# tikroeger/OF_DIS

Measured on AMD Instinct MI355X. Metric: frames/sec at 1024×436 op-point-2 (INT), higher is better.
Workload: dtype f32

## Files before the change

### of_dis_amd/csrc/ofdis_fused.hip

```cpp
#include <stdlib.h>

#include "ofdis_fused.h"

namespace ofdis {
namespace OFDIS_KNS {

constexpr int MW_LAG = 8;
constexpr int MW_MAX_ITERS = 8;
constexpr int MW_RING = 8;
constexpr int SP_LAG = 9;
constexpr int SP_MAX_ITERS = 6;


template <int NS, bool BRIGHT, int MODE, int NOC = 1>
__global__ __launch_bounds__(MODE == 2 ? 128 * SP_MAX_ITERS : (MODE == 1 ? 64 * MW_MAX_ITERS : 256))
__attribute__((amdgpu_waves_per_eu(NOC == 3 ? 2 : (MODE == 1 ? 3 : 1)))) void tv_fused_kernel(const FusedArgs a, const int R) {
  constexpr int U = 6;
  constexpr bool MW = MODE != 0;
  constexpr int MAXIT = MODE == 2 ? SP_MAX_ITERS : MW_MAX_ITERS;
  __shared__ float2 xring[MW ? (MAXIT - 1) * MW_RING * 64 : 1];
  __shared__ float sring[MODE == 2 ? SP_MAX_ITERS * 2 * SLOT_FLOATS * 64 : 1];
  __shared__ float2 wdring[MODE == 1 ? 6 * 64 : 1];
  __shared__ float2 obring[MODE == 1 ? 6 * 64 : 1];
  constexpr int PDW = 5, PDD = NOC == 3 ? 2 : 3;
  constexpr int PDU = MODE == 2 ? 4 : (MODE == 1 ? 3 : PDW);
  constexpr int LAG = MODE == 2 ? SP_LAG : MW_LAG;
  static_assert(2 * (NS - 1) + 1 < U, "slot ring too small for this many pipelined sweeps");
  static_assert(!MW || LAG >= PDU + 2 * (NS - 1) + 1, "a row must be published before the next iteration reads it");
  const int w = a.t.w, h = a.t.h;
  const int rw = a.S * w;
  const int lane = threadIdx.x & 63;
  const int wv = MW ? __builtin_amdgcn_readfirstlane(threadIdx.x >> 6) : 0;
  const int n_iters = MODE == 2 ? (int)(blockDim.x >> 7) : (MW ? (int)(blockDim.x >> 6) : 1);
  const bool is_solver = MODE == 2 && wv >= n_iters;
  const int it = MODE == 2 ? (is_solver ? wv - n_iters : wv) : wv;
  const bool do_p = MODE != 2 || !is_solver;
  const bool do_s = MODE != 2 || is_solver;
  const int wid = MW ? (int)blockIdx.x : __builtin_amdgcn_readfirstlane(blockIdx.x * 4 + (threadIdx.x >> 6));
  const int G = 64 / R;
  const int nstrips = a.t.nframes / a.S;
  const int s0 = wid * G;
  if (s0 >= nstrips) return;
  int fl = lane / R;
  const int jr = lane % R;
  const bool row_ok = (s0 + fl < nstrips) && (jr < h);
  if (s0 + fl >= nstrips) fl = nstrips - 1 - s0;
  const int j = jr < h ? jr : h - 1;
  const bool has_top = j > 0, has_bot = j < h - 1;
  const float omega = a.omega, qa = a.quarter_alpha, hd3 = a.half_delta_over3, hg3 = a.half_gamma_over3;
  auto from_prev = [&](float x) { return wave_from_prev(x); };
  auto from_next = [&](float x) { return wave_from_next(x); };

  const int nst = min(G, nstrips - s0);
  const size_t strip_recs = (size_t)rw * h;
  auto rsrc = [&](const float* base, int rec_floats) {
    return __builtin_amdgcn_make_buffer_rsrc((void*)(base + (size_t)s0 * strip_recs * rec_floats), 0,
                                             (int)(nst * strip_recs * rec_floats * 4), 0x00020000);
  };
  const __amdgpu_buffer_rsrc_t rsW = rsrc(a.wrec, 2), rsU = rsrc(a.uv, 2);
  const __amdgpu_buffer_rsrc_t rsD = rsrc(a.d8, 8);
  const __amdgpu_buffer_rsrc_t rsD1 = rsrc(a.d8 + (NOC == 3 ? (size_t)a.t.nframes * w * h * 8 : 0), 8);
  const __amdgpu_buffer_rsrc_t rsD2 = rsrc(a.d8 + (NOC == 3 ? (size_t)a.t.nframes * w * h * 16 : 0), 8);
  const int vrec = fl * (int)strip_recs + j;
  const int vo8 = vrec * 32, vo2 = vrec * 8;
  auto asf = [](unsigned u) { return __builtin_bit_cast(float, u); };

  const int npx = w * h;
  float2* const flow_row = a.flow_out
                               ? reinterpret_cast<float2*>(a.flow_out) + ((size_t)(s0 + fl) * a.S * npx + (size_t)j * w)
                               : nullptr;
  const bool aos_out = MODE != 2 && a.flow_out != nullptr;

  FRow W[6];
  FDer D[PDD][NOC];
  float uu[3], vv[3], sm[3];
  FSlot slot[6];
#pragma unroll
  for (int r = 0; r < 6; ++r) { W[r] = FRow{0, 0, 0, 0}; slot[r] = FSlot{1, 0, 1, 0, 0, 1, 1, 0, 0, 0, 0}; }
#pragma unroll
  for (int r = 0; r < 3; ++r) {
    uu[r] = vv[r] = 0.0f;
    sm[r] = 1.0f;
  }
#pragma unroll
  for (int r = 0; r < PDD; ++r)
#pragma unroll
    for (int c = 0; c < NOC; ++c) D[r][c] = FDer{0, 0, 0, 0, 0, 0, 0, 0};
  float ru[NS], rv[NS], ru2[NS], rv2[NS];
#pragma unroll
  for (int s = 0; s < NS; ++s) { ru[s] = rv[s] = ru2[s] = rv2[s] = 0.0f; }
  float ldx = 0.0f, ldy = 0.0f;
  float2 Wd[6], ob[U];
#pragma unroll
  for (int r = 0; r < 6; ++r) Wd[r] = make_float2(0.0f, 0.0f);
#pragma unroll
  for (int r = 0; r < U; ++r) ob[r] = make_float2(0.0f, 0.0f);
  int ox = 0, ooff = 0;

  auto ob_put = [&](int e, const float2& v) {
    if constexpr (MODE == 1) obring[lane * U + e] = v;
    else ob[e] = v;
  };
  auto ob_get = [&](int e) -> float2 {
    if constexpr (MODE == 1) return obring[lane * U + e];
    else return ob[e];
  };
  auto aos_emit = [&](int slot, bool flush, const float2& wq, float du, float dv, int c) {
    ob_put(slot, make_float2(wq.x + du, wq.y + dv));
    if (flush) {
      const int c0 = c - (U - 1);
      if (row_ok & (c0 >= 0) & (c < rw) & (ox >= U - 1)) {
        typedef float f4a8 __attribute__((ext_vector_type(4), aligned(8)));
        f4a8* d = reinterpret_cast<f4a8*>(flow_row + ooff + ox - (U - 1));
#pragma unroll
        for (int e = 0; e < U / 2; ++e) {
          const float2 p0 = ob_get(2 * e), p1 = ob_get(2 * e + 1);
          d[e] = f4a8{p0.x, p0.y, p1.x, p1.y};
        }
      } else if (row_ok & (c >= 0) & (c0 < rw)) {
#pragma unroll
        for (int e = 0; e < U; ++e) {
          const int ce = c0 + e;
          int xe = ox - (U - 1) + e, oe = ooff;
          if (xe < 0) { xe += w; oe -= npx; }
          if ((ce >= 0) & (ce < rw)) flow_row[oe + xe] = ob_get(e);
        }
      }
    }
    if (c >= 0) {
      ++ox;
      if (ox == w) { ox = 0; ooff += npx; }
    }
  };
  auto wrap_row = [&](int r) { r %= rw; return r < 0 ? r + rw : r; };
  auto wrap_col = [&](int c) { c %= w; return c < 0 ? c + w : c; };
  auto next_row = [&](int r) { return (r + 1 == rw) ? 0 : r + 1; };
  auto ring_uv = [&](FRow& r, int tau) {
    if (it == 0) {
      r.du = 0.0f; r.dv = 0.0f;
    } else {
      const float2 v = xring[((it - 1) * MW_RING + (tau & (MW_RING - 1))) * 64 + lane];
      r.du = v.x; r.dv = v.y;
    }
  };
  auto load_w = [&](FRow& r, int drow, int tau, bool zero_uv) {
    const int o = drow * h * 8;
    const auto t = __builtin_amdgcn_raw_buffer_load_b64(rsW, vo2, o, 0);
    const unsigned t0 = t[0], t1 = t[1];
    r.wx = asf(t0); r.wy = asf(t1);
    if constexpr (MODE == 0) {
      const auto q = __builtin_amdgcn_raw_buffer_load_b64(rsU, zero_uv ? 0x7ffffff0 : vo2, o, 0);
      const unsigned q0 = q[0], q1 = q[1];
      r.du = asf(q0); r.dv = asf(q1);
    }
  };
  auto load_d1 = [&](FDer& r, const __amdgpu_buffer_rsrc_t& rs, int o) {
    const auto lo = __builtin_amdgcn_raw_buffer_load_b128(rs, vo8, o, 0);
    const auto hi = __builtin_amdgcn_raw_buffer_load_b128(rs, vo8 + 16, o, 0);
    const unsigned l0 = lo[0], l1 = lo[1], l2 = lo[2], l3 = lo[3], h0 = hi[0], h1 = hi[1], h2 = hi[2], h3 = hi[3];
    r.ix = asf(l0); r.iz = asf(l1); r.ixx = asf(l2); r.ixz = asf(l3);
    r.iy = asf(h0); r.ixy = asf(h1); r.iyz = asf(h2); r.iyy = asf(h3);
  };
  auto load_d = [&](FDer (&r)[NOC], int drow) {
    const int o = drow * h * 32;
    load_d1(r[0], rsD, o);
    if constexpr (NOC == 3) {
      load_d1(r[1], rsD1, o);
      load_d1(r[2], rsD2, o);
    }
  };

  if constexpr (MW) {
    if (do_s && it < MAXIT - 1) {
#pragma unroll
      for (int q = 0; q < MW_RING; ++q) xring[(it * MW_RING + q) * 64 + lane] = make_float2(0.0f, 0.0f);
    }
    __syncthreads();
    for (int n = 0; n < it * LAG; ++n) __syncthreads();
  }
  if (do_p) {
    load_w(W[2], wrap_row(-1), -1, true);
    load_w(W[3], wrap_row(0), 0, true);
    if (PDW == 5) load_w(W[4], wrap_row(1), 1, true);
    if constexpr (MW) {
      ring_uv(W[2], -1);
      if (PDU == 4) ring_uv(W[3], 0);
    }
  }
  int rowW = wrap_row(PDW - 3);
  int tauW = PDW - 3;
  int rowD = wrap_row(PDD - 3);
  int srow = wrap_row(-3 - 2 * (NS - 1));
  int x2 = wrap_col(-1 - j);
  bool x1_last = (wrap_col(-2 - j) == w - 1);

  const int wtot = (MW ? 1 : a.n_inner) * rw;
  const int tend = (wtot - 1) + (h - 1) + 2 * (NS - 1);
  int ig = -3 - j - 2 * (NS - 1);
  bool first_w = !MW;
  int taus = -3 - 2 * (NS - 1);
  int taut = -3;
  for (int k0 = 0; k0 <= tend + 3; k0 += U) {
#pragma unroll
    for (int u = 0; u < U; ++u) {
      if (do_p) {
        load_w(W[(u + PDW) % 6], rowW, tauW, first_w);
        if constexpr (MW) ring_uv(W[(u + PDU) % 6], tauW - (PDW - PDU));
        rowW = next_row(rowW);
        ++tauW;
        load_d(D[(u + PDD) % PDD], rowD);
        rowD = next_row(rowD);
        {
          const FRow& r = W[(u + 3) % 6];
          uu[u % 3] = r.wx + r.du;
          vv[u % 3] = r.wy + r.dv;
        }
        const bool x2_last = (x2 == w - 1);
        {
          const float uc = uu[(u + 2) % 3], vc = vv[(u + 2) % 3];
          float ul = uu[(u + 1) % 3], vl = vv[(u + 1) % 3];
          float ur = uu[u % 3], vr = vv[u % 3];
          float ut = from_prev(uu[(u + 1) % 3]), vt = from_prev(vv[(u + 1) % 3]);
          float ub = from_next(uu[u % 3]), vb = from_next(vv[u % 3]);
          if (x2 == 0) { ul = uc; vl = vc; }
          if (x2_last) { ur = uc; vr = vc; }
          if (!has_top) { ut = uc; vt = vc; }
          if (!has_bot) { ub = uc; vb = vc; }
          const float ex = ur - ul, fx = vr - vl, ey = ub - ut, fy = vb - vt;
          sm[(u + 2) % 3] = fdiv_by_sqrt(qa, 0.25f * (ex * ex + ey * ey + fx * fx + fy * fy) + EPS_SMOOTH);
        }
        {
          const float sc = sm[(u + 1) % 3];
          const float s_r = sm[(u + 2) % 3];
          const float sh_c = x1_last ? 0.0f : sc + s_r;
          const FRow& rc = W[(u + 1) % 6];
          const FRow& rm = W[u % 6];
          const FRow& rp = W[(u + 2) % 6];
          float a11, a12, a22, b1, b2;
          if constexpr (NOC == 1) data_term_gray<BRIGHT>(D[(u + 1) % PDD][0], rc.du, rc.dv, hd3, hg3, a11, a12, a22, b1, b2);
          else data_term_rgb<BRIGHT>(D[(u + 1) % PDD], rc.du, rc.dv, hd3, hg3, a11, a12, a22, b1, b2);
          float udx, udy, ddx, ddy, sv_s;
          vertical_terms(udx, udy, ddx, ddy, sv_s, rc.wx, rc.wy, rm.wx, rm.wy, rp.wx, rp.wy, sc, sm[(u + 2) % 3]);
          const float sv_c = has_bot ? sv_s : 0.0f;
          const float sh_l = slot[u % 6].sh;
          const float sv_t = from_prev(slot[u % 6].sv);
          const float rdx = rp.wx - rc.wx, rdy = rp.wy - rc.wy;
          b1 -= sh_l * ldx;
          b2 -= sh_l * ldy;
          b1 += sh_c * rdx;
          b2 += sh_c * rdy;
          ldx = rdx; ldy = rdy;
          if constexpr (MODE == 0) Wd[(u + 1) % 6] = make_float2(rc.wx, rc.wy);
          if constexpr (MODE == 1) {
            if (it == n_iters - 1) wdring[((u + 1) % 6) * 64 + lane] = make_float2(rc.wx, rc.wy);
          }
          b1 -= sv_t * udx;
          b2 -= sv_t * udy;
          b1 += sv_c * ddx;
          b2 += sv_c * ddy;
          FSlot& o = slot[(u + 1) % 6];
          o.a11 = a11; o.a12 = a12; o.a22 = a22; o.b1 = b1; o.b2 = b2; o.sh = sh_c; o.sv = sv_c;
          o.dur = rp.du; o.dvr = rp.dv;
          o.hl = sh_l; o.vt = sv_t;
          if constexpr (MODE == 2) {
            float* sr = sring + ((it * 2 + ((taut + 1) & 1)) * SLOT_FLOATS) * 64 + lane;
            sr[0 * 64] = a11; sr[1 * 64] = a12; sr[2 * 64] = a22; sr[3 * 64] = b1; sr[4 * 64] = b2; sr[5 * 64] = sh_c;
            sr[6 * 64] = sv_c; sr[7 * 64] = rp.du; sr[8 * 64] = rp.dv; sr[9 * 64] = sh_l; sr[10 * 64] = sv_t;
          }
        }
        x1_last = x2_last;
        x2 = x2_last ? 0 : x2 + 1;
      }
      if (do_s) {
        if (MODE == 2 && taut > -3) {
          const float* sr = sring + ((it * 2 + (taut & 1)) * SLOT_FLOATS) * 64 + lane;
          FSlot& c = slot[u % 6];
          c.a11 = sr[0 * 64]; c.a12 = sr[1 * 64]; c.a22 = sr[2 * 64]; c.b1 = sr[3 * 64]; c.b2 = sr[4 * 64]; c.sh = sr[5 * 64];
          c.sv = sr[6 * 64]; c.dur = sr[7 * 64]; c.dvr = sr[8 * 64]; c.hl = sr[9 * 64]; c.vt = sr[10 * 64];
        }
        {
          FSlot& c = slot[u % 6];
          const float d = c.hl + c.sh + c.vt + c.sv;
          const float A11 = c.a22 + d, A22 = c.a11 + d;
          const float det = A11 * A22 - c.a12 * c.a12;
          const FDen dd = fden(det);
          c.a11 = fdiv_by(A11, dd);
          c.a22 = fdiv_by(A22, dd);
          c.a12 = -fdiv_by(c.a12, dd);
        }
        float nu[NS], nv[NS], ou[NS], ov[NS], rgu[NS], rgv[NS], wvt[NS], wsv[NS], s1[NS], s2[NS];
#pragma unroll
        for (int s = 0; s < NS; ++s) {
          const FSlot& c = slot[(u - 2 * s + 12) % 6];
          if (s == 0) {
            const FSlot& p = slot[(u + 5) % 6];
            ou[s] = p.dur; ov[s] = p.dvr;
            rgu[s] = c.dur; rgv[s] = c.dvr;
          } else {
            ou[s] = ru2[s - 1]; ov[s] = rv2[s - 1];
            rgu[s] = ru[s - 1]; rgv[s] = rv[s - 1];
          }
          wvt[s] = c.vt; wsv[s] = c.sv;
        }
        mul_pairs_from_prev(s1, s2, ru, rv, wvt);
#pragma unroll
        for (int s = 0; s < NS; ++s) {
          const FSlot& c = slot[(u - 2 * s + 12) % 6];
          s1[s] = c.sh * rgu[s] + s1[s];
          s2[s] = c.sh * rgv[s] + s2[s];
        }
        fmac_pairs_from_next(s1, s2, rgu, rgv, wsv);
#pragma unroll
        for (int s = 0; s < NS; ++s) {
          const FSlot& c = slot[(u - 2 * s + 12) % 6];
          const float lu = ru[s], lv = rv[s];
          const float t1 = s1[s] + c.b1, t2 = s2[s] + c.b2;
          const float B1 = c.hl * lu + t1, B2 = c.hl * lv + t2;
          nu[s] = ou[s] + omega * (c.a11 * B1 + c.a12 * B2 - ou[s]);
          nv[s] = ov[s] + omega * (c.a12 * B1 + c.a22 * B2 - ov[s]);
        }
        {
          if (!MW) {
            const int cw = ig + (PDW + 1 + 2 * (NS - 1));
            first_w = (cw < rw) | (cw >= wtot);
          }
          if (MW && it < n_iters - 1) {
            xring[(it * MW_RING + (taus & (MW_RING - 1))) * 64 + lane] = make_float2(nu[NS - 1], nv[NS - 1]);
          } else if (MODE == 2 && a.flow_out) {
            const auto q = __builtin_amdgcn_raw_buffer_load_b64(rsW, vo2, srow * h * 8, 0);
            const unsigned q0 = q[0], q1 = q[1];
            if (row_ok && ig >= 0 && ig < wtot)
              flow_row[ig] = make_float2(asf(q0) + nu[NS - 1], asf(q1) + nv[NS - 1]);
          } else if (MODE == 1 && a.flow_out) {
            aos_emit(u, u == U - 1, wdring[((u - 2 * (NS - 1) + 12) % 6) * 64 + lane], nu[NS - 1], nv[NS - 1], ig);
          } else if (!MW) {
            const u32x2 v = {__builtin_bit_cast(unsigned, nu[NS - 1]), __builtin_bit_cast(unsigned, nv[NS - 1])};
            const int lastc = ig - (wtot - rw);
            const bool on = row_ok & (ig >= 0) & (aos_out ? lastc < 0 : ig < wtot);
            __builtin_amdgcn_raw_buffer_store_b64(v, rsU, on ? vo2 : 0x7ffffff0, srow * h * 8, 0);
            if (aos_out) aos_emit(u, u == U - 1, Wd[(u - 2 * (NS - 1) + 12) % 6], nu[NS - 1], nv[NS - 1], lastc);
          } else if (row_ok && ig >= 0 && ig < wtot) {
            const u32x2 v = {__builtin_bit_cast(unsigned, nu[NS - 1]), __builtin_bit_cast(unsigned, nv[NS - 1])};
            __builtin_amdgcn_raw_buffer_store_b64(v, rsU, vo2, srow * h * 8, 0);
          }
        }
#pragma unroll
        for (int s = 0; s < NS; ++s) {
          ru2[s] = ru[s]; rv2[s] = rv[s];
          ru[s] = nu[s]; rv[s] = nv[s];
        }
      }
      srow = next_row(srow);
      ++ig;
      ++taus;
      ++taut;
      if constexpr (MW) mw_step_barrier();
    }
  }
  if constexpr (MW) {
    for (int n = 0; n < (n_iters - 1 - it) * LAG; ++n) __syncthreads();
  }
}

bool tv_fused_supported(const TvGeom& t, int iterations) {
  return ((t.noc == 1 || t.noc == 3) && t.h >= 2 && t.h <= 64 && t.w >= 16 && iterations >= 1 && iterations <= 3) ||
         tv_fused_tall_supported(t, iterations);
}

bool tv_fused_params_ok(float qa, float hd3, float hg3) {
  auto ok = [](float v) { return v == 0.0f || (v >= 1e-12f && v <= 1e12f); };
  return qa > 0.0f && ok(qa) && ok(hd3) && ok(hg3);
}

constexpr int MW_MAX_BATCH_FRAMES = 1024;

int tv_fused_mode(const FusedArgs& a, const FusedXcu* x) {
  const int h = a.t.h;
  if (h > 64) return 0;
  if (a.t.noc == 3)
    return (a.tp_pipe && a.S == 1 && a.n_inner >= 2 && a.n_inner <= MW_MAX_ITERS) ? 1 : 0;
  const int R = slot_rows(h);
  const int groups = (a.t.nframes + 64 / R - 1) / (64 / R);
  const int total = a.total_frames > 0 ? a.total_frames : a.t.nframes;
  if (x && x->xbuf && x->err && a.S == 1 && a.n_inner >= 2 && groups <= x->max_groups && total <= MW_MAX_BATCH_FRAMES) return 3;
  const bool mw = a.S == 1 && a.n_inner >= 2 && a.n_inner <= MW_MAX_ITERS && groups <= a.mw_max_groups &&
                  (total <= MW_MAX_BATCH_FRAMES || a.mw_max_groups >= (1 << 30));
  if (mw) return (a.split && a.n_inner <= SP_MAX_ITERS) ? 2 : 1;
  return (a.tp_pipe && a.n_inner >= 2 && a.n_inner <= MW_MAX_ITERS) ? 1 : 0;
}

hipError_t launch_tv_fused(const FusedArgs& a, hipStream_t s, bool* wrote_flow, const FusedXcu* x) {
  if (wrote_flow) *wrote_flow = false;
  if (!tv_fused_supported(a.t, a.iterations) || a.n_inner < 1 || a.S < 1 || a.t.nframes % a.S != 0 ||
      !tv_fused_params_ok(a.quarter_alpha, a.half_delta_over3, a.half_gamma_over3))
    return hipErrorInvalidValue;
  const int h = a.t.h;
  if (h > 64) {
    if (wrote_flow) *wrote_flow = a.flow_out != nullptr;
    return launch_tv_fused_tall(a, s, a.tall_group);
  }
  const int R = slot_rows(h);
  const int G = 64 / R;
  const int nstrips = a.t.nframes / a.S;
  const int waves = (nstrips + G - 1) / G;
  const int blocks = (waves + 3) / 4;
  const bool bright = a.half_delta_over3 != 0.0f;
  const int mode = tv_fused_mode(a, x);
  if (wrote_flow) *wrote_flow = a.flow_out != nullptr;
  if (mode == 3) return launch_tv_fused_xcu(a, *x, waves, R, s);
  if (a.t.noc == 3 && a.S != 1) return hipErrorInvalidValue;
  const dim3 gd(mode == 0 ? blocks : waves), bd(mode == 0 ? 256 : 64 * mode * a.n_inner);
  auto launch = [&](auto NOC, auto MODE) {
    with_constant<1, 2, 3>(a.iterations, [&](auto NS) {
      with_constant<false, true>(bright, [&](auto BRIGHT) {
        hipLaunchKernelGGL((tv_fused_kernel<decltype(NS)::value, decltype(BRIGHT)::value, decltype(MODE)::value, decltype(NOC)::value>),
                           gd, bd, 0, s, a, R);
      });
    });
  };
  using std::integral_constant;
  if (a.t.noc == 3)
    with_constant<1, 0>(mode, [&](auto MODE) { launch(integral_constant<int, 3>{}, MODE); });
  else
    with_constant<2, 1, 0>(mode, [&](auto MODE) { launch(integral_constant<int, 1>{}, MODE); });
  return hipGetLastError();
}

}
}
```

Baseline: 1.606 million.

## Write MODE-1 flow output directly via buffer stores, drop LDS staging rings

For the multi-wave MODE 1 path, the wdring and obring LDS staging buffers are removed. The last-iteration wave now reloads the warp row from global memory and stores each finished flow pixel straight to the output through a buffer resource, computing the frame/column offset arithmetically. Non-writer waves get a zero-sized resource so their loads and stores are masked off. The ring_uv branch on it==0 is replaced with a branchless mask. This cuts LDS traffic and footprint and the batched AoS flush logic, at the cost of an extra global load per row and narrower, scattered stores.

```diff
diff --git a/of_dis_amd/csrc/ofdis_fused.hip b/of_dis_amd/csrc/ofdis_fused.hip
--- a/of_dis_amd/csrc/ofdis_fused.hip
+++ b/of_dis_amd/csrc/ofdis_fused.hip
@@ -20,8 +20,6 @@
   constexpr int MAXIT = MODE == 2 ? SP_MAX_ITERS : MW_MAX_ITERS;
   __shared__ float2 xring[MW ? (MAXIT - 1) * MW_RING * 64 : 1];
   __shared__ float sring[MODE == 2 ? SP_MAX_ITERS * 2 * SLOT_FLOATS * 64 : 1];
-  __shared__ float2 wdring[MODE == 1 ? 6 * 64 : 1];
-  __shared__ float2 obring[MODE == 1 ? 6 * 64 : 1];
   constexpr int PDW = 5, PDD = NOC == 3 ? 2 : 3;
   constexpr int PDU = MODE == 2 ? 4 : (MODE == 1 ? 3 : PDW);
   constexpr int LAG = MODE == 2 ? SP_LAG : MW_LAG;
@@ -53,9 +51,9 @@
 
   const int nst = min(G, nstrips - s0);
   const size_t strip_recs = (size_t)rw * h;
-  auto rsrc = [&](const float* base, int rec_floats) {
+  auto rsrc = [&](const float* base, int rec_floats, bool on = true) {
     return __builtin_amdgcn_make_buffer_rsrc((void*)(base + (size_t)s0 * strip_recs * rec_floats), 0,
-                                             (int)(nst * strip_recs * rec_floats * 4), 0x00020000);
+                                             on ? (int)(nst * strip_recs * rec_floats * 4) : 0, 0x00020000);
   };
   const __amdgpu_buffer_rsrc_t rsW = rsrc(a.wrec, 2), rsU = rsrc(a.uv, 2);
   const __amdgpu_buffer_rsrc_t rsD = rsrc(a.d8, 8);
@@ -69,7 +67,15 @@
   float2* const flow_row = a.flow_out
                                ? reinterpret_cast<float2*>(a.flow_out) + ((size_t)(s0 + fl) * a.S * npx + (size_t)j * w)
                                : nullptr;
-  const bool aos_out = MODE != 2 && a.flow_out != nullptr;
+  const bool aos_out = MODE == 0 && a.flow_out != nullptr;
+  const bool writer = MODE == 1 && it == n_iters - 1 && a.flow_out != nullptr;
+  constexpr int XD = 3 + 2 * (NS - 1);
+  static_assert(XD < 16, "a lane's finished column and the producer's are in the same or in consecutive frames: w >= 16 > XD");
+  const __amdgpu_buffer_rsrc_t rsF = rsrc(a.flow_out, 2, writer), rsQ = rsrc(a.wrec, 2, writer);
+  const int fo8 = (fl * (int)strip_recs + j * w) * 8;
+  float2 wq[2] = {make_float2(0.0f, 0.0f), make_float2(0.0f, 0.0f)};
+  const unsigned uvmask = it == 0 ? 0u : ~0u;
+  const int uvring = (it == 0 ? 0 : it - 1) * MW_RING;
 
   FRow W[6];
   FDer D[PDD][NOC];
@@ -97,14 +103,8 @@
   for (int r = 0; r < U; ++r) ob[r] = make_float2(0.0f, 0.0f);
   int ox = 0, ooff = 0;
 
-  auto ob_put = [&](int e, const float2& v) {
-    if constexpr (MODE == 1) obring[lane * U + e] = v;
-    else ob[e] = v;
-  };
-  auto ob_get = [&](int e) -> float2 {
-    if constexpr (MODE == 1) return obring[lane * U + e];
-    else return ob[e];
-  };
+  auto ob_put = [&](int e, const float2& v) { ob[e] = v; };
+  auto ob_get = [&](int e) -> float2 { return ob[e]; };
   auto aos_emit = [&](int slot, bool flush, const float2& wq, float du, float dv, int c) {
     ob_put(slot, make_float2(wq.x + du, wq.y + dv));
     if (flush) {
@@ -136,12 +136,9 @@
   auto wrap_col = [&](int c) { c %= w; return c < 0 ? c + w : c; };
   auto next_row = [&](int r) { return (r + 1 == rw) ? 0 : r + 1; };
   auto ring_uv = [&](FRow& r, int tau) {
-    if (it == 0) {
-      r.du = 0.0f; r.dv = 0.0f;
-    } else {
-      const float2 v = xring[((it - 1) * MW_RING + (tau & (MW_RING - 1))) * 64 + lane];
-      r.du = v.x; r.dv = v.y;
-    }
+    const float2 v = xring[(uvring + (tau & (MW_RING - 1))) * 64 + lane];
+    r.du = asf(__builtin_bit_cast(unsigned, v.x) & uvmask);
+    r.dv = asf(__builtin_bit_cast(unsigned, v.y) & uvmask);
   };
   auto load_w = [&](FRow& r, int drow, int tau, bool zero_uv) {
     const int o = drow * h * 8;
@@ -204,6 +201,11 @@
 #pragma unroll
     for (int u = 0; u < U; ++u) {
       if (do_p) {
+        if constexpr (MODE == 1) {
+          const auto q = __builtin_amdgcn_raw_buffer_load_b64(rsQ, vo2, next_row(srow) * h * 8, 0);
+          const unsigned q0 = q[0], q1 = q[1];
+          wq[(u + 1) % 2] = make_float2(asf(q0), asf(q1));
+        }
         load_w(W[(u + PDW) % 6], rowW, tauW, first_w);
         if constexpr (MW) ring_uv(W[(u + PDU) % 6], tauW - (PDW - PDU));
         rowW = next_row(rowW);
@@ -251,9 +253,6 @@
           b2 += sh_c * rdy;
           ldx = rdx; ldy = rdy;
           if constexpr (MODE == 0) Wd[(u + 1) % 6] = make_float2(rc.wx, rc.wy);
-          if constexpr (MODE == 1) {
-            if (it == n_iters - 1) wdring[((u + 1) % 6) * 64 + lane] = make_float2(rc.wx, rc.wy);
-          }
           b1 -= sv_t * udx;
           b2 -= sv_t * udy;
           b1 += sv_c * ddx;
@@ -331,8 +330,12 @@
             const unsigned q0 = q[0], q1 = q[1];
             if (row_ok && ig >= 0 && ig < wtot)
               flow_row[ig] = make_float2(asf(q0) + nu[NS - 1], asf(q1) + nv[NS - 1]);
-          } else if (MODE == 1 && a.flow_out) {
-            aos_emit(u, u == U - 1, wdring[((u - 2 * (NS - 1) + 12) % 6) * 64 + lane], nu[NS - 1], nv[NS - 1], ig);
+          } else if (MODE == 1 && writer) {
+            const float2 wf = wq[u % 2];
+            const int xf = x2 < XD ? x2 + (w - XD) : x2 - XD;
+            const bool on = row_ok & ((unsigned)ig < (unsigned)rw);
+            const u32x2 v = {__builtin_bit_cast(unsigned, wf.x + nu[NS - 1]), __builtin_bit_cast(unsigned, wf.y + nv[NS - 1])};
+            __builtin_amdgcn_raw_buffer_store_b64(v, rsF, on ? fo8 + __mul24(ig, h * 8) - __mul24(xf, (h - 1) * 8) : 0x7ffffff0, 0, 0);
           } else if (!MW) {
             const u32x2 v = {__builtin_bit_cast(unsigned, nu[NS - 1]), __builtin_bit_cast(unsigned, nv[NS - 1])};
             const int lastc = ig - (wtot - rw);
```

Result: no change. 1.611 million (median of 2 runs) (+0.4%).
